# FraPria/proovread

Hardware: AMD Instinct MI355X
Metric: corrected long-read Mbases/sec per node (higher is better)
Workload: dtype int32

## Files before the change

### include/prgpu.h

```cpp
#ifndef PRGPU_H
#define PRGPU_H
#include <stdint.h>
#ifdef __cplusplus
extern "C" {
#endif

enum {
    PR_OK = 0,
    PR_ERR_ARG = -1,
    PR_ERR_HIP = -2,
    PR_ERR_SAM = -3,
    PR_ERR_NOSEQ = -4,
    PR_ERR_BIN_RANGE = -5,
    PR_ERR_DIV0 = -6,
    PR_ERR_CIGAR = -7,
    PR_ERR_BEYOND_REF = -8,
    PR_ERR_CAPACITY = -9,
    PR_ERR_UNSUPPORTED = -10,
};

const char *pr_last_error(void);
const char *pr_version(void);

typedef struct pr_ctx pr_ctx;
// ... 224 lines not shown
int pr_seed_map(const pr_seed_index *h, const pr_seed_opts *o, const uint8_t *sr_seq, const int64_t *sr_off,
                int n_sr, int n_threads, pr_seed_tasks *out);
void pr_seed_tasks_free(pr_seed_tasks *t);
int pr_seed_index_occ(const pr_seed_index *h, const uint8_t *s, int n, int64_t *count);
int pr_seed_index_digest(const pr_seed_index *h, uint64_t *out6);
int pr_seed_index_koff(const pr_seed_index *h, uint64_t *koff, uint64_t *ksplit);
int pr_seed_gpu_index_koff(pr_ctx *ctx, uint64_t *koff, uint64_t *ksplit);
int pr_seed_smem(const pr_seed_index *h, const uint8_t *q, int len, int x, int64_t min_intv, int32_t *start,
                 int32_t *end, int64_t *occ, int cap, int *n_out);
int pr_seed_gpu_upload(pr_ctx *ctx, const pr_seed_index *h);
int pr_seed_gpu_map(pr_ctx *ctx, const pr_seed_opts *o, const uint8_t *sr_seq, const int64_t *sr_off, int n_sr,
                    pr_seed_tasks *out, int32_t *status);
int pr_seed_gpu_index_build(pr_ctx *ctx, const uint8_t *lr_seq, const int64_t *lr_off, int n_lr);
int pr_seed_gpu_index_digest(pr_ctx *ctx, uint64_t *out6);
int pr_seed_gpu_index_last_ms(pr_ctx *ctx, double *ms);
int pr_seed_gpu_seed_count(pr_ctx *ctx, int64_t *n);
int pr_seed_gpu_seeds(pr_ctx *ctx, pr_seed_tasks *out);
int pr_seed_gpu_pass2_reads(pr_ctx *ctx, int64_t *n);
int pr_seed_gpu_pass_reads(pr_ctx *ctx, int64_t *n4);
int pr_seed_gpu_last_ms(pr_ctx *ctx, double *ms);
int pr_seed_gpu_phase_ticks(pr_ctx *ctx, uint64_t *ticks4);
int pr_seed_gpu_lane_ticks(pr_ctx *ctx, uint64_t *ticks6);
int pr_seed_gpu_occ_ticks(pr_ctx *ctx, uint64_t *ticks3);
int pr_seed_gpu_pass2_ticks(pr_ctx *ctx, uint64_t *t7);
int pr_seed_gpu_pass2_ms(pr_ctx *ctx, double *ms);
int pr_seed_map_device_caps(const pr_seed_index *h, const pr_seed_opts *o, const uint8_t *sr_seq,
                            const int64_t *sr_off, int n_sr, int n_threads, pr_seed_tasks *out, int32_t *status);
int pr_seed_map_device_pass1(const pr_seed_index *h, const pr_seed_opts *o, const uint8_t *sr_seq,
                             const int64_t *sr_off, int n_sr, int budget, pr_seed_tasks *out, int32_t *status,
                             int32_t *hits);

typedef struct pr_iter_batch {
    pr_sw_batch sw;
    const int64_t *task_lr_off;
    const uint8_t *lr_qual;
    const uint8_t *ref_seq;
} pr_iter_batch;
int pr_iter_upload(pr_ctx *ctx, const pr_iter_batch *b);
int pr_iter_upload_gpu_seeds(pr_ctx *ctx, const pr_iter_batch *b);
int pr_iter_launch(pr_ctx *ctx, const pr_sw_opts *o, const pr_cns_params *p);
int pr_iter_download(pr_ctx *ctx, pr_cns_out *out);
int pr_fmt_chim_lines(int32_t n_lr, const char *names, const int64_t *name_off, const int32_t *nchim,
                      const int64_t *chim_off, const int32_t *chim, char **text, int64_t *len, int64_t *n_lines);
int pr_iter_download_range(pr_ctx *ctx, int32_t first, int32_t n, pr_cns_out *out);
int pr_iter_bounds(pr_ctx *ctx, int32_t *n_lr, int64_t *n_task, pr_cns_bounds *bd);
int pr_iter_alignment_stats(pr_ctx *ctx, int64_t *n_aln, int64_t *sum_ncig, int64_t *sum_lseq);
// ... 171 lines not shown
```

### proovread_amd/csrc/seed_api.cpp

```cpp
#include <algorithm>
#include <climits>
#include <cstdio>
#include <cstdlib>
#include <cstring>
#include <vector>

#include "ctx.h"
#include "seed_index_dev.h"
#include "seed_plan.h"

static int seed_text4(pr_ctx *c, seedc::IndexView &v, hipStream_t s) {
    int rc = c->sd[SI_TEXT4].ensure((size_t)ix_pack4_words(v.n_text) * 8);
    if (rc) return rc;
    const int e = ix_pack4_launch(v.text, v.n_text, c->sd[SI_TEXT4].as<uint64_t>(), s);
    if (e) return set_error(PR_ERR_HIP, "text packing: %s", hipGetErrorString((hipError_t)e));
    v.text4 = c->sd[SI_TEXT4].as<uint64_t>();
    v.walk_nw = v.n_text > ((int64_t)64 << 24) ? 1 : 4;
    if (const char *w = getenv("PRGPU_SEED_WALK_NW"))
        v.walk_nw = atoi(w) == 1 ? 1 : 4;
    return 0;
}

static int upload_blk_fr(pr_ctx *c, seedc::IndexView &v, const int64_t *cstart, const int64_t *off, int n_lr,
                         int64_t l_pac, int64_t n_text, hipStream_t s) {
// ... 380 lines not shown
                          : 0;
}

int map_buffers(SeedMap &M, const pr_seed_opts *o, const uint8_t *sr_seq, bool in_sb_seq, const int64_t *sr_off) {
    pr_ctx *c = M.c;
    DevBuf *D = M.D;
    SeedDev &K = M.K;
    const int n_sr = M.n_sr;
    hipStream_t s = M.s;
    int rc;
    K.dp = nullptr;
    if (seedc::seed_flt_min_score(*o, M.qmax) >= 0) {
        if ((rc = D[SB_DP].ensure((size_t)M.waves * 2 * 201 * 64 * sizeof(int16_t)))) return rc;
        K.dp = D[SB_DP].as<int16_t>();
    }
    const int64_t scratch = std::max<int64_t>(M.waves * 64 * K.stride, M.lanes2 * seedc::scratch_bytes(M.caps));
    const int64_t nb = n_sr ? sr_off[n_sr] : 0;
    const int64_t slot_bytes = (int64_t)M.caps.out * (int64_t)sizeof(pr_seed_task);
    c->seed_sr_bases = nb;
    if ((!in_sb_seq && (rc = upload(D[SB_SEQ], sr_seq, (size_t)nb, s))) || (rc = upload(D[SB_OFF], sr_off, (size_t)n_sr + 1, s)) ||
        (rc = D[SB_SCRATCH].ensure((size_t)scratch)) ||
        (rc = D[SB_OUT].ensure((size_t)(std::min<int64_t>(M.chunk, n_sr) * slot_bytes + 16))) ||
        (rc = D[SB_NOUT].ensure((size_t)n_sr * 4 + 16)) || (rc = D[SB_STATUS].ensure((size_t)n_sr * 4 + 16)) ||
        (rc = D[SB_NEXT].ensure(256)) || (rc = D[SB_PRE].ensure(((size_t)n_sr + 1) * 8)) ||
        (rc = D[SB_DENSE].ensure(sizeof(pr_seed_task))) || (M.occ_words && (rc = D[SB_OCC].ensure((size_t)M.occ_words * 8))))
        return rc;
    K.sr_seq = D[SB_SEQ].as<uint8_t>();
    K.sr_off = D[SB_OFF].as<int64_t>();
    K.out = D[SB_OUT].as<pr_seed_task>();
    K.n_out = D[SB_NOUT].as<int32_t>();
    K.status = D[SB_STATUS].as<int32_t>();
    K.next = D[SB_NEXT].as<int32_t>();
    K.prof = reinterpret_cast<unsigned long long *>(D[SB_NEXT].as<uint8_t>() + 64);
    K.occ = seedc::OccPool{D[SB_OCC].as<uint64_t>(), reinterpret_cast<unsigned long long *>(K.next + 4), M.occ_words};
    HIPCHK(hipMemsetAsync(K.next, 0, 256, s));
    return 0;
}

int pass1(SeedMap &M, int64_t r0, int64_t r1, std::vector<int32_t> &redo, seedp::Flagged &f) {
    DevBuf *D = M.D;
    SeedDev &K = M.K;
    hipStream_t s = M.s;
    int rc;
    K.caps = M.small;
    K.caps.budget = M.budget;
    K.stride = seedc::scratch_bytes(M.small);
    K.n_lanes = M.waves;
    K.batch = 64;
    K.scratch = D[SB_SCRATCH].as<uint8_t>();
    K.rlist = nullptr;
    K.n_list = 0;
    K.out0 = r0;
    K.n_sr = r1;
    int32_t start = (int32_t)r0;
    const char *lpt = getenv("PRGPU_SEED_LPT");
    if (lpt && lpt[0] == '1') {
        int32_t *order = nullptr;
        if ((rc = D[SB_ORDER].ensure(seed_order_bytes(r1 - r0)))) return rc;
// ... 278 lines not shown
    if (!c || !ticks4) return set_error(PR_ERR_ARG, "null arg");
    if (!c->sd[SB_NEXT].p) return set_error(PR_ERR_ARG, "no pr_seed_gpu_map launch yet");
    HIPCHK(hipSetDevice(c->device));
    HIPCHK(hipMemcpy(ticks4, c->sd[SB_NEXT].as<uint8_t>() + 64, 32, hipMemcpyDeviceToHost));
    return 0;
}

extern "C" int pr_seed_gpu_lane_ticks(pr_ctx *c, uint64_t *ticks6) {
    if (!c || !ticks6) return set_error(PR_ERR_ARG, "null arg");
    if (!c->sd[SB_NEXT].p) return set_error(PR_ERR_ARG, "no pr_seed_gpu_map launch yet");
    HIPCHK(hipSetDevice(c->device));
    HIPCHK(hipMemcpy(ticks6, c->sd[SB_NEXT].as<uint8_t>() + 64 + 4 * 8, 48, hipMemcpyDeviceToHost));
    return 0;
}

extern "C" int pr_seed_gpu_pass2_ticks(pr_ctx *c, uint64_t *t7) {
    if (!c || !t7) return set_error(PR_ERR_ARG, "null arg");
    if (!c->sd[SB_NEXT].p) return set_error(PR_ERR_ARG, "no pr_seed_gpu_map launch yet");
    HIPCHK(hipSetDevice(c->device));
    HIPCHK(hipMemcpy(t7, c->sd[SB_NEXT].as<uint8_t>() + 64 + 13 * 8, 56, hipMemcpyDeviceToHost));
    return 0;
}

extern "C" int pr_seed_gpu_occ_ticks(pr_ctx *c, uint64_t *ticks3) {
    if (!c || !ticks3) return set_error(PR_ERR_ARG, "null arg");
    if (!c->sd[SB_NEXT].p) return set_error(PR_ERR_ARG, "no pr_seed_gpu_map launch yet");
    HIPCHK(hipSetDevice(c->device));
    HIPCHK(hipMemcpy(ticks3, c->sd[SB_NEXT].as<uint8_t>() + 64 + 10 * 8, 24, hipMemcpyDeviceToHost));
    return 0;
}
```

### proovread_amd/csrc/seed_chain.h

```cpp
#pragma once
#include "seed_core.h"

#if defined(__HIP_DEVICE_COMPILE__)
#define SCC_SYNC()                                              \
    do {                                                        \
        __builtin_amdgcn_fence(__ATOMIC_RELEASE, "wavefront");  \
        __builtin_amdgcn_wave_barrier();                        \
        __builtin_amdgcn_fence(__ATOMIC_ACQUIRE, "wavefront");  \
    } while (0)
#define SCC_LANES \
    for (int lane = (int)__builtin_amdgcn_mbcnt_hi(~0u, __builtin_amdgcn_mbcnt_lo(~0u, 0u)), go_ = 1; go_; go_ = 0)
#define SCC_END SCC_SYNC()
#define SCC_ADD(p, v) __hip_atomic_fetch_add(p, v, __ATOMIC_RELAXED, __HIP_MEMORY_SCOPE_WORKGROUP)
#define SCC_OR(p, v) __hip_atomic_fetch_or(p, v, __ATOMIC_RELAXED, __HIP_MEMORY_SCOPE_WORKGROUP)
namespace prgpu {
namespace seedc {
template <class T> __device__ inline T scc_cas(T *p, T c, T v) {
    __hip_atomic_compare_exchange_strong(p, &c, v, __ATOMIC_RELAXED, __ATOMIC_RELAXED, __HIP_MEMORY_SCOPE_WORKGROUP);
    return c;
}
}
}
#define SCC_CAS(p, c, v) ::prgpu::seedc::scc_cas(p, c, v)
#define SCC_NOW() __builtin_amdgcn_s_memrealtime()
#define SCC_STAT(L, k) ((void)0)
#else
#define SCC_STAT(L, k) (++(L).sv[k])
#define SCC_LANES for (int lane = 0; lane < 64; ++lane)
#define SCC_END ((void)0)
namespace prgpu {
namespace seedc {
template <class T> inline T scc_add(T *p, T v) { const T o = *p; *p = (T)(o + v); return o; }
template <class T> inline T scc_or(T *p, T v) { const T o = *p; *p = (T)(o | v); return o; }
template <class T> inline T scc_cas(T *p, T c, T v) { const T o = *p; if (o == c) *p = v; return o; }
}
}
#define SCC_ADD(p, v) ::prgpu::seedc::scc_add(p, v)
#define SCC_OR(p, v) ::prgpu::seedc::scc_or(p, v)
#define SCC_CAS(p, c, v) ::prgpu::seedc::scc_cas(p, c, v)
#define SCC_NOW() 0ULL
#endif

namespace prgpu {
namespace seedc {

constexpr int32_t OCC_MAX = 16384;
struct OccPool {
    uint64_t *w;
    unsigned long long *cursor;
    int64_t cap;
};
SC_HD constexpr int64_t occ_words(int n) { return (int64_t)n + (n + 1) / 2; }
SC_HD const uint32_t *occ_ql(const uint64_t *hfr, int n) { return reinterpret_cast<const uint32_t *>(hfr + n); }
SC_HD int32_t occ_words_per_read(bool lazy) { return lazy ? 384 : 3072; }

SC_HD int occ_taken(const pr_seed_opts &O, int64_t np) {
    const int64_t step = np > O.max_occ ? np / O.max_occ : 1;
// ... 65 lines not shown
    *first = w0;
    *n_occ = n;
    return 0;
}

template <int S, int HT, int CH>
struct ChainLds {
    static_assert(S % 8 == 0 && S < 32768 && CH % 64 == 0 && (HT & (HT - 1)) == 0, "slot indices are int16");
    static constexpr int SEEDS = S, RANGES = HT / 2;
    uint64_t hfr[S];
    uint32_t ql[S];
    int16_t nx[S];
    int16_t chead[S], ctail[S], cn[S];
    int16_t cnx[S];
    uint16_t cidx[S];
    int16_t ts[S];
    union {
        struct {
            int32_t key[HT];
            int16_t head[HT], tail[HT];
            uint64_t hfr[CH];
            uint32_t ql[CH];
            int16_t idx[CH];
            uint8_t own[CH];
        } ch;
        struct {
            int16_t pl[S];
            int16_t sch[S];
            int16_t kept[S];
            int16_t fm[S];
            int16_t kb[S], ke[S], kw[S];
        } po;
    } u;
    int32_t cnt[64], cur[64];
    int32_t sv[16];
    uint32_t mk[2][4];
};
enum {
    SV_ERR = 0, SV_NRG, SV_NP, SV_NK, SV_LARGE, SV_DROP, SV_NO, SV_STEP, SV_NS, SV_NC,
    SV_TIES, SV_INS_HEAD, SV_INS_MID, SV_INS_TAIL, SV_WR_LT
};

SC_HD uint32_t range_hash(int32_t key) { return (uint32_t)key * 0x9E3779B1u; }

template <int S, int HT, int CH>
SC_HD int chain_read(const IndexView &I, const pr_seed_opts &O, ChainLds<S, HT, CH> &L, const uint64_t *g_hfr,
                     const uint32_t *g_ql, int n, int len, int sid, pr_seed_task *out, int cap_out, int *n_out,
                     unsigned long long *ticks = nullptr, int lim_seeds = S, int lim_chains = S) {
    *n_out = 0;
    lim_seeds = lim_seeds < S ? lim_seeds : S;
    lim_chains = lim_chains < S ? lim_chains : S;
    if (n > OCC_MAX) return SC_OVER_SEEDS;
    if (n <= 0) return 0;
    unsigned long long t_last = ticks ? SCC_NOW() : 0ULL;
    (void)t_last;
#define SCC_TICK(k)                                     \
    do {                                                \
        if (ticks) {                                    \
            const unsigned long long t_ = SCC_NOW();    \
            ticks[k] += t_ - t_last;                    \
            t_last = t_;                                \
        }                                               \
    } while (0)
    const int64_t l_pac = I.l_pac;
    auto rbeg = [&L](int e) -> int64_t { return (int64_t)(L.hfr[e] >> FR_RID_BITS); };
    auto qb = [&L](int e) -> int { return (int)(L.ql[e] & 0xFFFFu); };
    auto sl = [&L](int e) -> int { return (int)(L.ql[e] >> 16); };

    SCC_LANES {
        if (lane < 16) L.sv[lane] = 0;
        if (lane < 8) L.mk[lane >> 2][lane & 3] = 0u;
        for (int k = lane; k < HT; k += 64) L.u.ch.key[k] = -1;
    }
    SCC_END;
    for (int c0 = 0; c0 < n && !L.sv[SV_ERR]; c0 += CH) {
        const int m = n - c0 < CH ? n - c0 : CH;
        SCC_LANES { L.cnt[lane] = 0; }
        SCC_END;
        SCC_LANES {
            for (int e = lane; e < m; e += 64) {
                const uint64_t v = g_hfr[c0 + e];
                L.u.ch.hfr[e] = v;
                L.u.ch.ql[e] = g_ql[c0 + e];
                const int rid = (int)(v & ((1u << FR_RID_BITS) - 1u));
                const int32_t key = rid * 2 + ((int64_t)(v >> FR_RID_BITS) >= l_pac ? 1 : 0);
                const int o = (int)(range_hash(key) >> 26);
                L.u.ch.own[e] = (uint8_t)o;
                SCC_ADD(&L.cnt[o], 1);
            }
            for (int e = m + lane; e < ((m + 7) & ~7); e += 64) L.u.ch.own[e] = 255;
        }
        SCC_END;
        SCC_LANES {
            int x = 0;
            for (int t = 0; t < lane; ++t) x += L.cnt[t];
            L.cur[lane] = x;
        }
        SCC_END;
        SCC_LANES {
            int c = L.cur[lane];
            for (int e0 = 0; e0 < m; e0 += 8) {
                uint64_t w;
                __builtin_memcpy(&w, L.u.ch.own + e0, 8);
#pragma unroll
                for (int u = 0; u < 8; ++u)
                    if ((int)((w >> (8 * u)) & 0xFF) == lane) L.u.ch.idx[c++] = (int16_t)(e0 + u);
            }
        }
        SCC_END;
        SCC_LANES {
            const int first = L.cur[lane], mine = L.cnt[lane];
            for (int t = 0; t < mine; ++t) {
                const int e = L.u.ch.idx[first + t];
                const uint64_t v = L.u.ch.hfr[e];
                const uint32_t qlv = L.u.ch.ql[e];
                const int64_t rb = (int64_t)(v >> FR_RID_BITS);
                const int rid = (int)(v & ((1u << FR_RID_BITS) - 1u));
                const int32_t key = rid * 2 + (rb >= l_pac ? 1 : 0);
                const int qbe = (int)(qlv & 0xFFFFu), sle = (int)(qlv >> 16);
                uint32_t h = range_hash(key) & (uint32_t)(HT - 1);
                bool found = false, claimed = false;
                for (int probe = 0; probe < HT; ++probe) {
                    const int32_t kk = L.u.ch.key[h];
                    if (kk == key) { found = true; break; }
                    if (kk == -1) {
                        const int32_t old = SCC_CAS(&L.u.ch.key[h], (int32_t)-1, key);
                        if (old == -1) { claimed = true; break; }
                        if (old == key) { found = true; break; }
                    }
                    h = (h + 1) & (uint32_t)(HT - 1);
                }
                if (claimed && SCC_ADD(&L.sv[SV_NRG], 1) >= HT / 2) claimed = false;
// ... 47 lines not shown
                L.cn[c] = 1;
                L.cidx[c] = (uint16_t)(c0 + e);
                if (!found) {
                    L.u.ch.head[h] = L.u.ch.tail[h] = (int16_t)c;
                    L.cnx[c] = -1;
                } else if (at < 0) {
                    L.cnx[c] = L.u.ch.head[h];
                    L.u.ch.head[h] = (int16_t)c;
                    SCC_STAT(L, SV_INS_HEAD);
                } else {
                    const int nxc = L.cnx[at];
                    L.cnx[c] = (int16_t)nxc;
                    L.cnx[at] = (int16_t)c;
                    if (nxc < 0) {
                        L.u.ch.tail[h] = (int16_t)c;
                        SCC_STAT(L, SV_INS_TAIL);
                    } else {
                        SCC_STAT(L, SV_INS_MID);
                    }
                }
            }
        }
        SCC_END;
    }
    if (L.sv[SV_ERR]) return L.sv[SV_ERR];
    SCC_TICK(0);
    const int ncv = L.sv[SV_NC];
    SCC_LANES {
        for (int c = lane; c < ncv; c += 64) {
            int64_t qe = 0, re = 0;
            int wq = 0, wr = 0;
            for (int k = L.chead[c]; k >= 0; k = L.nx[k]) {
                const int q0 = qb(k), ln = sl(k);
                const int64_t r0 = rbeg(k);
                if (q0 >= qe) wq += ln;
                else if (q0 + ln > qe) wq += (int)(q0 + ln - qe);
                qe = qe > q0 + ln ? qe : q0 + ln;
                if (r0 >= re) wr += ln;
                else if (r0 + ln > re) wr += (int)(r0 + ln - re);
                re = re > r0 + ln ? re : r0 + ln;
            }
            int w = wr < wq ? wr : wq;
            if (wr < wq) SCC_STAT(L, SV_WR_LT);
            w = w < 32767 ? w : 32767;
            L.cnx[c] = (int16_t)w;
        }
    }
    SCC_END;
    SCC_LANES {
        for (int c = lane; c < ncv; c += 64) {
            const int w = L.cnx[c];
            if (w >= O.min_chain_weight) {
                const int m = SCC_ADD(&L.sv[SV_NP], 1);
                L.u.po.pl[m] = (int16_t)c;
                L.u.po.kw[m] = (int16_t)w;
            }
        }
    }
    SCC_END;
    const int nch = L.sv[SV_NP];
    const bool keep_all = O.drop_ratio <= 0;
    SCC_LANES {
        for (int m = lane; m < nch; m += 64) {
            const int c = L.u.po.pl[m], w = L.u.po.kw[m];
            const int64_t ps = rbeg(L.chead[c]);
            const int ix = L.cidx[c];
            int rank = 0;
            for (int j = 0; j < nch; ++j) {
                const int wj = L.u.po.kw[j];
                if (wj > w) ++rank;
                else if (wj == w) {
                    const int cj = L.u.po.pl[j];
                    const int64_t pj = rbeg(L.chead[cj]);
                    rank += (pj < ps || (pj == ps && (int)L.cidx[cj] < ix)) ? 1 : 0;
                    if (pj == ps && cj != c) SCC_STAT(L, SV_TIES);
                }
            }
            L.u.po.sch[rank] = (int16_t)c;
            L.u.po.kept[rank] = keep_all ? 3 : 0;
        }
    }
    SCC_END;
    if (nch > 0 && !keep_all) {
        SCC_LANES {
            if (lane == 0) {
                const int c = L.u.po.sch[0], hd = L.chead[c], tl = L.ctail[c];
                const int w0 = L.cnx[c];
                L.u.po.kb[0] = (int16_t)qb(hd);
                L.u.po.ke[0] = (int16_t)(qb(tl) + sl(tl));
                L.u.po.kw[0] = (int16_t)w0;
                L.u.po.fm[0] = -1;
                L.u.po.kept[0] = 3;
                L.sv[SV_NK] = 1;
                L.sv[SV_LARGE] = L.sv[SV_DROP] = 0;
                L.sv[SV_STEP] = 0;
            }
        }
        SCC_END;
        for (int i = 1; i < nch; ++i) {
            const int ci = L.u.po.sch[i], hi = L.chead[ci], ti = L.ctail[ci];
            const int bi = qb(hi), ei = qb(ti) + sl(ti), wi = L.cnx[ci];
            for (int k0 = 0; k0 < L.sv[SV_NK] && !L.sv[SV_DROP]; k0 += 64) {
                const int set = L.sv[SV_STEP] & 1;
                SCC_LANES {
                    const int k = k0 + lane;
                    if (k < L.sv[SV_NK]) {
                        const int bj = L.u.po.kb[k], ej = L.u.po.ke[k], wj = L.u.po.kw[k];
                        const int bmax = bj > bi ? bj : bi;
                        const int emin = ej < ei ? ej : ei;
                        if (emin > bmax) {
                            const int li = ei - bi, lj = ej - bj;
                            const int minl = li < lj ? li : lj;
                            if (emin - bmax >= minl * O.mask_level && minl < O.max_chain_gap) {
                                SCC_OR(&L.mk[set][lane >> 5], 1u << (lane & 31));
                                if (wi < wj * O.drop_ratio && wj - wi >= O.min_seed_len << 1)
                                    SCC_OR(&L.mk[set][2 + (lane >> 5)], 1u << (lane & 31));
                            }
                        }
                    }
                }
                SCC_END;
                SCC_LANES {
                    const uint64_t ov = (uint64_t)L.mk[set][0] | ((uint64_t)L.mk[set][1] << 32);
                    const uint64_t br = (uint64_t)L.mk[set][2] | ((uint64_t)L.mk[set][3] << 32);
                    const int last = br ? ctz64(br) : 63;
                    const uint64_t seen = ov & (last >= 63 ? ~0ull : ((2ull << last) - 1ull));
                    if (((seen >> lane) & 1ull) && L.u.po.fm[k0 + lane] < 0) L.u.po.fm[k0 + lane] = (int16_t)i;
                    if (lane == 63) {
                        if (seen) L.sv[SV_LARGE] = 1;
                        if (br) L.sv[SV_DROP] = 1;
                        L.sv[SV_STEP] = set ^ 1;
                        L.mk[set ^ 1][0] = L.mk[set ^ 1][1] = L.mk[set ^ 1][2] = L.mk[set ^ 1][3] = 0u;
                    }
                }
                SCC_END;
            }
            SCC_LANES {
                if (lane == 0) {
                    if (!L.sv[SV_DROP]) {
                        const int nk = L.sv[SV_NK];
                        L.u.po.kb[nk] = (int16_t)bi;
                        L.u.po.ke[nk] = (int16_t)ei;
                        L.u.po.kw[nk] = (int16_t)wi;
                        L.u.po.fm[nk] = -1;
                        L.u.po.kept[i] = L.sv[SV_LARGE] ? 2 : 3;
                        L.sv[SV_NK] = nk + 1;
                    }
                    L.sv[SV_LARGE] = L.sv[SV_DROP] = 0;
                }
            }
            SCC_END;
        }
        SCC_LANES {
            for (int k = lane; k < L.sv[SV_NK]; k += 64)
                if (L.u.po.fm[k] >= 0) L.u.po.kept[L.u.po.fm[k]] = 1;
        }
        SCC_END;
    }
    SCC_TICK(1);
    SCC_LANES {
        if (lane == 0) {
            int no = 0, nkept = 0;
            for (int i = 0; i < nch; ++i) {
                if (L.u.po.kept[i] == 0) {
                    L.u.po.kb[i] = -1;
                    continue;
                }
                L.u.po.kb[i] = (int16_t)no;
                L.u.po.ke[i] = (int16_t)nkept++;
                no += L.cn[L.u.po.sch[i]];
            }
            L.sv[SV_NO] = no;
        }
    }
    SCC_END;
    const int no = L.sv[SV_NO];
    if (no > cap_out) return SC_OVER_OUT;
    SCC_LANES {
        for (int i = lane; i < nch; i += 64) {
            int t = L.u.po.kb[i];
            if (t < 0) continue;
            for (int k = L.chead[L.u.po.sch[i]]; k >= 0; k = L.nx[k], ++t) {
                L.ts[t] = (int16_t)k;
                L.u.po.pl[t] = (int16_t)i;
            }
        }
    }
    SCC_END;
    SCC_LANES {
        for (int t = lane; t < no; t += 64) {
            const int i = L.u.po.pl[t], k = L.ts[t];
            const int c = L.u.po.sch[i], first = L.u.po.kb[i], cnn = L.cn[c];
            const int hd = L.chead[c];
            const int ln = sl(k);
            int rank = 0;
            int64_t r0 = INT64_MAX, r1 = INT64_MIN;
            for (int u = first; u < first + cnn; ++u) {
                const int ku = L.ts[u];
                const int qu = qb(ku), lu = sl(ku);
// ... 6 lines not shown
            }
            const int rid = (int)(L.hfr[hd] & ((1u << FR_RID_BITS) - 1u));
            const bool rev = rbeg(hd) >= l_pac;
            const int64_t lo0 = I.lr_off[rid], lo1 = I.lr_off[rid + 1];
            const int64_t Lr = lo1 - lo0;
            const int64_t cs = rev ? l_pac + (l_pac - lo1) : lo0;
            r0 -= cs;
            r1 -= cs;
            pr_seed_task tk;
            tk.sr = sid;
            tk.lr = rid;
            tk.strand = rev ? 1 : 0;
            tk.qbeg = qb(k);
            tk.rbeg = (int32_t)(rbeg(k) - cs);
            tk.slen = ln;
            tk.rmax0 = (int32_t)(r0 > 0 ? r0 : 0);
            tk.rmax1 = (int32_t)(r1 < Lr ? r1 : Lr);
            tk.chain = L.u.po.ke[i];
            tk.rank = rank;
            out[first + rank] = tk;
        }
    }
    SCC_END;
    SCC_TICK(2);
#undef SCC_TICK
    *n_out = no;
    return 0;
}

using ChainLdsSmall = ChainLds<512, 512, 256>;
using ChainLdsLarge = ChainLds<1536, 2048, 256>;

struct ChainHost {
    ChainLdsSmall a;
    ChainLdsLarge b;
    uint64_t pool[occ_words(OCC_MAX)];
};
template <class LA, class LB>
SC_HD int map_read_chain2(const IndexView &I, const pr_seed_opts &O, Scratch &S, LA &La, LB &Lb, uint64_t *pool,
                          int64_t pool_words, const uint8_t *q, int len, int sid, pr_seed_task *out, int cap_out,
                          int *n_out) {
    *n_out = 0;
    if (seed_flt_min_score(O, len) >= 0) return map_read(I, O, S, q, len, sid, out, cap_out, n_out);
    int err = S.hend ? build_starts(I, S, q, len) : build_occ(I, S, q, len);
    if (err) return err;
    int nm = 0, nocc = 0;
    unsigned long long cursor = 0;
// ... 32 lines not shown
```

### proovread_amd/csrc/seed_kernels.hip

```cpp
#include <hip/hip_runtime.h>

#include <rocprim/device/device_radix_sort.hpp>

#include "seed_chain.h"
#include "seed_core.h"
#include "seed_dev.h"

namespace prgpu {

#ifndef SEED_WAVES_DEF
#define SEED_WAVES_DEF 4
#endif
#ifndef SEED_LMAX_DEF
#define SEED_LMAX_DEF 1024
#endif
constexpr int SEED_WAVES = SEED_WAVES_DEF;
constexpr int SEED_LMAX = SEED_LMAX_DEF;
#ifndef SEED_MINB
#define SEED_MINB 4
#endif
#ifndef SEED_WAVE_MINB
#define SEED_WAVE_MINB SEED_MINB
#endif
#ifndef OCC_U
// ... 953 lines not shown
    int nb = 0;
    const hipError_t e = walk_nw == 1 ? hipOccupancyMaxActiveBlocksPerMultiprocessor(&nb, seed_wave_kernel<1>, 64 * SEED_WAVES, 0)
                                      : hipOccupancyMaxActiveBlocksPerMultiprocessor(&nb, seed_wave_kernel<4>, 64 * SEED_WAVES, 0);
    if (e != hipSuccess || nb < 1)
        nb = 2;
    return nb * SEED_WAVES;
}

int seed_launch(const SeedDev &D, void *stream) {
    if (D.n_list <= 0) return 0;
    const int64_t blocks = (D.n_lanes + SEED_WAVES - 1) / SEED_WAVES;
    if (D.V.walk_nw == 1)
        hipLaunchKernelGGL(seed_wave_kernel<1>, dim3((unsigned)blocks), dim3(64 * SEED_WAVES), 0, (hipStream_t)stream, D);
    else
        hipLaunchKernelGGL(seed_wave_kernel<4>, dim3((unsigned)blocks), dim3(64 * SEED_WAVES), 0, (hipStream_t)stream, D);
    return (int)hipGetLastError();
}

template <class LDS, bool SECOND>
__global__ void __launch_bounds__(64) seed_chain_kernel(SeedDev D) {
    __shared__ LDS L;
    const int lane = threadIdx.x;
    const int64_t nlim = D.rlist ? D.n_list : D.n_sr - D.out0;
    unsigned long long ct[3] = {0ULL, 0ULL, 0ULL};
    for (;;) {
        int j0 = 0;
        if (lane == 0) j0 = atomicAdd(D.next + (SECOND ? 2 : 1), 64);
        j0 = __shfl(j0, 0, 64);
        if (j0 >= nlim) {
            if (D.prof && lane == 0)
                for (int k = 0; k < 3; ++k) atomicAdd(&D.prof[4 + 3 + k], ct[k] * 64ULL);
            break;
        }
        int my_i = -1, my_n = 0, my_len = 0;
        if (j0 + lane < nlim) {
            const int i = D.rlist ? D.rlist[j0 + lane] : (int)(D.out0 + j0 + lane);
            const int len = (int)(D.sr_off[i + 1] - D.sr_off[i]);
            const int n = D.n_out[i];
            if (len > 0 && D.status[i] == 0 && seedc::seed_flt_min_score(D.O, len) < 0 && (SECOND ? n < 0 : n > 0))
                my_i = i, my_n = SECOND ? -n - 1 : n, my_len = len;
        }
        unsigned long long todo = __ballot(my_i >= 0);
        while (todo) {
            const int src = __ffsll((long long)todo) - 1;
            todo &= todo - 1;
            const int i = __shfl(my_i, src, 64), n = __shfl(my_n, src, 64), len = __shfl(my_len, src, 64);
            pr_seed_task *slots = D.out + (int64_t)(i - D.out0) * D.caps.out;
            const int64_t w0 = *reinterpret_cast<const int64_t *>(slots);
            __builtin_amdgcn_wave_barrier();
            const uint64_t *hfr = D.occ.w + w0;
            int nt = 0;
            const int err = seedc::chain_read(D.V, D.O, L, hfr, seedc::occ_ql(hfr, n), n, len, i, slots, D.caps.out, &nt,
                                              D.prof && lane == 0 ? ct : nullptr, D.caps.seeds, D.caps.chains);
            if (lane == 0) {
// ... 67 lines not shown
```

### proovread_amd/seed.py

```python
from __future__ import annotations

import ctypes as C

import numpy as np

from . import _abi


class SeedOpts(C.Structure):
    _fields_ = [("min_seed_len", C.c_int), ("min_chain_weight", C.c_int), ("w", C.c_int),
                ("split_factor", C.c_double), ("split_width", C.c_int), ("max_mem_intv", C.c_int),
                ("max_occ", C.c_int), ("drop_ratio", C.c_double), ("max_chain_gap", C.c_int),
                ("mask_level", C.c_double), ("a", C.c_int), ("o_del", C.c_int), ("e_del", C.c_int),
                ("o_ins", C.c_int), ("e_ins", C.c_int), ("b", C.c_int)]


class SeedTask(C.Structure):
    _fields_ = [(k, C.c_int32) for k in ("sr", "lr", "strand", "qbeg", "rbeg", "slen", "rmax0", "rmax1",
                                          "chain", "rank")]


class SeedTasks(C.Structure):
    _fields_ = [("n", C.c_int64), ("t", C.POINTER(SeedTask))]

# ... 172 lines not shown
def _phase_ms(L, ctx) -> dict:
    t = np.zeros(4, np.uint64)
    _abi.check(L.pr_seed_gpu_phase_ticks(ctx.h, t.ctypes.data), "pr_seed_gpu_phase_ticks")
    n2 = C.c_int64()
    _abi.check(L.pr_seed_gpu_pass2_reads(ctx.h, C.byref(n2)), "pr_seed_gpu_pass2_reads")
    out = {k: round(float(v) / 1e5, 1) for k, v in
           zip(("occ_table", "lane_phase_and_pass2_smems", "pass2_chaining", "pass2_filter_out"), t)}
    out["pass2_reads"] = n2.value
    if hasattr(L, "pr_seed_gpu_pass_reads"):
        pr = np.zeros(4, np.int64)
        L.pr_seed_gpu_pass_reads.argtypes = [C.c_void_p, C.c_void_p]
        _abi.check(L.pr_seed_gpu_pass_reads(ctx.h, pr.ctypes.data), "pr_seed_gpu_pass_reads")
        out["pass_reads"] = dict(zip(("pass1b_lane", "pass1b_wave", "pass2", "later"), (int(v) for v in pr)))
    lt = np.zeros(6, np.uint64)
    L.pr_seed_gpu_lane_ticks.argtypes = [C.c_void_p, C.c_void_p]
    _abi.check(L.pr_seed_gpu_lane_ticks(ctx.h, lt.ctypes.data), "pr_seed_gpu_lane_ticks")
    out["pass1_lane_ms_summed"] = {k: round(float(v) / 1e5, 1) for k, v in
                                   zip(("smem_pass", "reseeding", "y_seeds_sort", "chaining", "chain_flt", "output"), lt)}
    if hasattr(L, "pr_seed_gpu_occ_ticks"):
        ot = np.zeros(3, np.uint64)
        L.pr_seed_gpu_occ_ticks.argtypes = [C.c_void_p, C.c_void_p]
        _abi.check(L.pr_seed_gpu_occ_ticks(ctx.h, ot.ctypes.data), "pr_seed_gpu_occ_ticks")
        out["occ_table_parts"] = {k: round(float(v) / 1e5, 1) for k, v in zip(("starts", "hits", "count_table"), ot)}
    if hasattr(L, "pr_seed_gpu_pass2_ticks"):
        t2 = np.zeros(7, np.uint64)
        L.pr_seed_gpu_pass2_ticks.argtypes = [C.c_void_p, C.c_void_p]
        _abi.check(L.pr_seed_gpu_pass2_ticks(ctx.h, t2.ctypes.data), "pr_seed_gpu_pass2_ticks")
        out["pass2_parts"] = {"one_lane_reads": int(t2[0])}
        out["pass2_parts"].update({k: round(float(v) / 1e5, 1) for k, v in
                                   zip(("chain_wave", "chain_one_lane", "chain_flt", "max_read_occ_table",
                                        "max_read_smems", "max_read"), t2[1:])})
    p2 = C.c_double()
    _abi.check(L.pr_seed_gpu_pass2_ms(ctx.h, C.byref(p2)), "pr_seed_gpu_pass2_ms")
    out["pass2_wall_ms"] = round(p2.value, 1)
    return out


def _map_gpu(L, ctx, sr_seq, sr_off, opts, allow_flagged, keep_on_device=False):
    opts = opts or default_opts()
    sr_seq = np.ascontiguousarray(sr_seq, np.uint8)
    sr_off = np.ascontiguousarray(sr_off, np.int64)
    st = np.zeros(max(1, len(sr_off) - 1), np.int32)
    if keep_on_device:
        rc = L.pr_seed_gpu_map(ctx.h, C.byref(opts), sr_seq.ctypes.data, sr_off.ctypes.data, len(sr_off) - 1,
                               None, st.ctypes.data)
        if rc != 0 and not (allow_flagged and rc == -9):
# ... 45 lines not shown
```

Measured before the change: 239.0.

## Replace LDS atomics and serial loops in wave chaining with ballot/readlane primitives

Adds lane-register, ballot, readlane broadcast and prefix-scan primitives to the wave-level chaining kernel. It uses them to rewrite the owner bucketing (ballot match instead of LDS atomic counting and byte scans, with the next chunk prefetched into registers), the rank sort (keys broadcast across lanes instead of O(n^2) per-lane LDS reads), the drop pass (first 64 kept chains held in registers and masks built by ballot instead of LDS mask words and barriers), and the output-base computation (wave scan instead of a lane-0 serial loop). It also adds finer profiling tick counters and a host API to read them. The aim is to cut LDS traffic, barriers and serial single-lane work in the chaining phase, at the cost of more register pressure and more complex control flow.

```diff
diff --git a/include/prgpu.h b/include/prgpu.h
--- a/include/prgpu.h
+++ b/include/prgpu.h
@@ -270,6 +270,7 @@
 int pr_seed_gpu_phase_ticks(pr_ctx *ctx, uint64_t *ticks4);
 int pr_seed_gpu_lane_ticks(pr_ctx *ctx, uint64_t *ticks6);
 int pr_seed_gpu_occ_ticks(pr_ctx *ctx, uint64_t *ticks3);
+int pr_seed_gpu_chain_ticks(pr_ctx *ctx, uint64_t *ticks7);
 int pr_seed_gpu_pass2_ticks(pr_ctx *ctx, uint64_t *t7);
 int pr_seed_gpu_pass2_ms(pr_ctx *ctx, double *ms);
 int pr_seed_map_device_caps(const pr_seed_index *h, const pr_seed_opts *o, const uint8_t *sr_seq,
diff --git a/proovread_amd/csrc/seed_api.cpp b/proovread_amd/csrc/seed_api.cpp
--- a/proovread_amd/csrc/seed_api.cpp
+++ b/proovread_amd/csrc/seed_api.cpp
@@ -426,7 +426,7 @@
         (rc = D[SB_SCRATCH].ensure((size_t)scratch)) ||
         (rc = D[SB_OUT].ensure((size_t)(std::min<int64_t>(M.chunk, n_sr) * slot_bytes + 16))) ||
         (rc = D[SB_NOUT].ensure((size_t)n_sr * 4 + 16)) || (rc = D[SB_STATUS].ensure((size_t)n_sr * 4 + 16)) ||
-        (rc = D[SB_NEXT].ensure(256)) || (rc = D[SB_PRE].ensure(((size_t)n_sr + 1) * 8)) ||
+        (rc = D[SB_NEXT].ensure(512)) || (rc = D[SB_PRE].ensure(((size_t)n_sr + 1) * 8)) ||
         (rc = D[SB_DENSE].ensure(sizeof(pr_seed_task))) || (M.occ_words && (rc = D[SB_OCC].ensure((size_t)M.occ_words * 8))))
         return rc;
     K.sr_seq = D[SB_SEQ].as<uint8_t>();
@@ -437,7 +437,7 @@
     K.next = D[SB_NEXT].as<int32_t>();
     K.prof = reinterpret_cast<unsigned long long *>(D[SB_NEXT].as<uint8_t>() + 64);
     K.occ = seedc::OccPool{D[SB_OCC].as<uint64_t>(), reinterpret_cast<unsigned long long *>(K.next + 4), M.occ_words};
-    HIPCHK(hipMemsetAsync(K.next, 0, 256, s));
+    HIPCHK(hipMemsetAsync(K.next, 0, 512, s));
     return 0;
 }
 
@@ -762,6 +762,14 @@
     return 0;
 }
 
+extern "C" int pr_seed_gpu_chain_ticks(pr_ctx *c, uint64_t *ticks7) {
+    if (!c || !ticks7) return set_error(PR_ERR_ARG, "null arg");
+    if (!c->sd[SB_NEXT].p) return set_error(PR_ERR_ARG, "no pr_seed_gpu_map launch yet");
+    HIPCHK(hipSetDevice(c->device));
+    HIPCHK(hipMemcpy(ticks7, c->sd[SB_NEXT].as<uint8_t>() + 64 + 24 * 8, 56, hipMemcpyDeviceToHost));
+    return 0;
+}
+
 extern "C" int pr_seed_gpu_occ_ticks(pr_ctx *c, uint64_t *ticks3) {
     if (!c || !ticks3) return set_error(PR_ERR_ARG, "null arg");
     if (!c->sd[SB_NEXT].p) return set_error(PR_ERR_ARG, "no pr_seed_gpu_map launch yet");
diff --git a/proovread_amd/csrc/seed_chain.h b/proovread_amd/csrc/seed_chain.h
--- a/proovread_amd/csrc/seed_chain.h
+++ b/proovread_amd/csrc/seed_chain.h
@@ -24,6 +24,34 @@
 #define SCC_CAS(p, c, v) ::prgpu::seedc::scc_cas(p, c, v)
 #define SCC_NOW() __builtin_amdgcn_s_memrealtime()
 #define SCC_STAT(L, k) ((void)0)
+namespace prgpu {
+namespace seedc {
+__device__ inline int scc_lane() { return (int)__builtin_amdgcn_mbcnt_hi(~0u, __builtin_amdgcn_mbcnt_lo(~0u, 0u)); }
+template <class T> struct LaneReg {
+    T v;
+    __device__ T &at(int) { return v; }
+    __device__ const T &at(int) const { return v; }
+};
+template <class F> __device__ inline uint64_t scc_ballot(F f) { return __builtin_amdgcn_ballot_w64(f(scc_lane()) ? true : false); }
+__device__ inline int scc_bcast(const LaneReg<int> &r, int src) { return __builtin_amdgcn_readlane(r.v, src); }
+__device__ inline uint64_t scc_bcast(const LaneReg<uint64_t> &r, int src) {
+    const uint32_t lo = (uint32_t)__builtin_amdgcn_readlane((int)(uint32_t)r.v, src);
+    const uint32_t hi = (uint32_t)__builtin_amdgcn_readlane((int)(uint32_t)(r.v >> 32), src);
+    return (uint64_t)hi << 32 | lo;
+}
+template <class F> __device__ inline int scc_scan(LaneReg<int> &ex, F f) {
+    const int lane = scc_lane(), v = f(lane);
+    int x = v;
+#pragma unroll
+    for (int d = 1; d < 64; d <<= 1) {
+        const int y = __builtin_amdgcn_ds_bpermute((lane - d) << 2, x);
+        if (lane >= d) x += y;
+    }
+    ex.v = x - v;
+    return __builtin_amdgcn_readlane(x, 63);
+}
+}
+}
 #else
 #define SCC_STAT(L, k) (++(L).sv[k])
 #define SCC_LANES for (int lane = 0; lane < 64; ++lane)
@@ -33,6 +61,24 @@
 template <class T> inline T scc_add(T *p, T v) { const T o = *p; *p = (T)(o + v); return o; }
 template <class T> inline T scc_or(T *p, T v) { const T o = *p; *p = (T)(o | v); return o; }
 template <class T> inline T scc_cas(T *p, T c, T v) { const T o = *p; if (o == c) *p = v; return o; }
+template <class T> struct LaneReg {
+    T v[64];
+    T &at(int lane) { return v[lane]; }
+    const T &at(int lane) const { return v[lane]; }
+};
+template <class F> inline uint64_t scc_ballot(F f) {
+    uint64_t m = 0;
+    for (int lane = 0; lane < 64; ++lane) m |= f(lane) ? 1ull << lane : 0ull;
+    return m;
+}
+inline int scc_bcast(const LaneReg<int> &r, int src) { return r.v[src & 63]; }
+inline uint64_t scc_bcast(const LaneReg<uint64_t> &r, int src) { return r.v[src & 63]; }
+template <class F> inline int scc_scan(LaneReg<int> &ex, F f) {
+    int v[64], x = 0;
+    for (int lane = 0; lane < 64; ++lane) v[lane] = f(lane);
+    for (int lane = 0; lane < 64; ++lane) ex.v[lane] = x, x += v[lane];
+    return x;
+}
 }
 }
 #define SCC_ADD(p, v) ::prgpu::seedc::scc_add(p, v)
@@ -144,7 +190,6 @@
             uint64_t hfr[CH];
             uint32_t ql[CH];
             int16_t idx[CH];
-            uint8_t own[CH];
         } ch;
         struct {
             int16_t pl[S];
@@ -156,12 +201,13 @@
     } u;
     int32_t cnt[64], cur[64];
     int32_t sv[16];
-    uint32_t mk[2][4];
 };
 enum {
-    SV_ERR = 0, SV_NRG, SV_NP, SV_NK, SV_LARGE, SV_DROP, SV_NO, SV_STEP, SV_NS, SV_NC,
+    SV_ERR = 0, SV_NRG, SV_NP, SV_NS, SV_NC,
     SV_TIES, SV_INS_HEAD, SV_INS_MID, SV_INS_TAIL, SV_WR_LT
 };
+
+enum { CT_LOAD = 0, CT_LANES, CT_WEIGHTS, CT_SORT, CT_DROP, CT_BASE, CT_TASKS, CT_N };
 
 SC_HD uint32_t range_hash(int32_t key) { return (uint32_t)key * 0x9E3779B1u; }
 
@@ -191,45 +237,81 @@
 
     SCC_LANES {
         if (lane < 16) L.sv[lane] = 0;
-        if (lane < 8) L.mk[lane >> 2][lane & 3] = 0u;
         for (int k = lane; k < HT; k += 64) L.u.ch.key[k] = -1;
     }
     SCC_END;
+    constexpr int G = CH / 64;
+    LaneReg<uint64_t> nh[G];
+    LaneReg<uint32_t> nq[G];
+    auto fetch = [&](int c0) {
+        SCC_LANES {
+#pragma unroll
+            for (int g = 0; g < G; ++g) {
+                const int e = c0 + g * 64 + lane;
+                nh[g].at(lane) = e < n ? g_hfr[e] : 0ull;
+                nq[g].at(lane) = e < n ? g_ql[e] : 0u;
+            }
+        }
+    };
+    fetch(0);
     for (int c0 = 0; c0 < n && !L.sv[SV_ERR]; c0 += CH) {
         const int m = n - c0 < CH ? n - c0 : CH;
-        SCC_LANES { L.cnt[lane] = 0; }
+        LaneReg<int> own[G], pos[G], add[G], cur;
+        SCC_LANES {
+            L.cnt[lane] = 0;
+#pragma unroll
+            for (int g = 0; g < G; ++g) {
+                const int e = g * 64 + lane;
+                own[g].at(lane) = -1;
+                pos[g].at(lane) = add[g].at(lane) = 0;
+                if (e < m) {
+                    const uint64_t v = nh[g].at(lane);
+                    L.u.ch.hfr[e] = v;
+                    L.u.ch.ql[e] = nq[g].at(lane);
+                    const int rid = (int)(v & ((1u << FR_RID_BITS) - 1u));
+                    const int32_t key = rid * 2 + ((int64_t)(v >> FR_RID_BITS) >= l_pac ? 1 : 0);
+                    own[g].at(lane) = (int)(range_hash(key) >> 26);
+                }
+            }
+        }
+        SCC_END;
+        if (c0 + CH < n) fetch(c0 + CH);
+#pragma unroll
+        for (int g = 0; g < G; ++g) {
+            if (g * 64 >= m) break;
+            uint64_t bit[6];
+#pragma unroll
+            for (int b = 0; b < 6; ++b) bit[b] = scc_ballot([&](int lane) { return (own[g].at(lane) >> b) & 1; });
+            const uint64_t valid = scc_ballot([&](int lane) { return own[g].at(lane) >= 0; });
+            SCC_LANES {
+                const int o = own[g].at(lane);
+                if (o >= 0) {
+                    uint64_t same = valid;
+#pragma unroll
+                    for (int b = 0; b < 6; ++b) same &= ((o >> b) & 1) ? bit[b] : ~bit[b];
+                    const int before = __builtin_popcountll(same & ((1ull << lane) - 1ull));
+                    pos[g].at(lane) = L.cnt[o] + before;
+                    add[g].at(lane) = before ? 0 : __builtin_popcountll(same);
+                }
+            }
+            SCC_END;
+            SCC_LANES {
+                if (add[g].at(lane)) L.cnt[own[g].at(lane)] += add[g].at(lane);
+            }
+            SCC_END;
+        }
+        scc_scan(cur, [&](int lane) { return (int)L.cnt[lane]; });
+        SCC_LANES { L.cur[lane] = cur.at(lane); }
         SCC_END;
         SCC_LANES {
-            for (int e = lane; e < m; e += 64) {
-                const uint64_t v = g_hfr[c0 + e];
-                L.u.ch.hfr[e] = v;
-                L.u.ch.ql[e] = g_ql[c0 + e];
-                const int rid = (int)(v & ((1u << FR_RID_BITS) - 1u));
-                const int32_t key = rid * 2 + ((int64_t)(v >> FR_RID_BITS) >= l_pac ? 1 : 0);
-                const int o = (int)(range_hash(key) >> 26);
-                L.u.ch.own[e] = (uint8_t)o;
-                SCC_ADD(&L.cnt[o], 1);
-            }
-            for (int e = m + lane; e < ((m + 7) & ~7); e += 64) L.u.ch.own[e] = 255;
+#pragma unroll
+            for (int g = 0; g < G; ++g) {
+                const int o = own[g].at(lane);
+                if (o >= 0) L.u.ch.idx[L.cur[o] + pos[g].at(lane)] = (int16_t)(g * 64 + lane);
+            }
         }
         SCC_END;
-        SCC_LANES {
-            int x = 0;
-            for (int t = 0; t < lane; ++t) x += L.cnt[t];
-            L.cur[lane] = x;
-        }
-        SCC_END;
-        SCC_LANES {
-            int c = L.cur[lane];
-            for (int e0 = 0; e0 < m; e0 += 8) {
-                uint64_t w;
-                __builtin_memcpy(&w, L.u.ch.own + e0, 8);
-#pragma unroll
-                for (int u = 0; u < 8; ++u)
-                    if ((int)((w >> (8 * u)) & 0xFF) == lane) L.u.ch.idx[c++] = (int16_t)(e0 + u);
-            }
-        }
-        SCC_END;
+        SCC_TICK(CT_LOAD);
         SCC_LANES {
             const int first = L.cur[lane], mine = L.cnt[lane];
             for (int t = 0; t < mine; ++t) {
@@ -323,9 +405,9 @@
             }
         }
         SCC_END;
+        SCC_TICK(CT_LANES);
     }
     if (L.sv[SV_ERR]) return L.sv[SV_ERR];
-    SCC_TICK(0);
     const int ncv = L.sv[SV_NC];
     SCC_LANES {
         for (int c = lane; c < ncv; c += 64) {
@@ -354,128 +436,163 @@
             if (w >= O.min_chain_weight) {
                 const int m = SCC_ADD(&L.sv[SV_NP], 1);
                 L.u.po.pl[m] = (int16_t)c;
-                L.u.po.kw[m] = (int16_t)w;
+                L.ts[m] = (int16_t)w;
             }
         }
     }
     SCC_END;
     const int nch = L.sv[SV_NP];
+    SCC_TICK(CT_WEIGHTS);
     const bool keep_all = O.drop_ratio <= 0;
-    SCC_LANES {
-        for (int m = lane; m < nch; m += 64) {
-            const int c = L.u.po.pl[m], w = L.u.po.kw[m];
-            const int64_t ps = rbeg(L.chead[c]);
-            const int ix = L.cidx[c];
-            int rank = 0;
-            for (int j = 0; j < nch; ++j) {
-                const int wj = L.u.po.kw[j];
-                if (wj > w) ++rank;
-                else if (wj == w) {
-                    const int cj = L.u.po.pl[j];
-                    const int64_t pj = rbeg(L.chead[cj]);
-                    rank += (pj < ps || (pj == ps && (int)L.cidx[cj] < ix)) ? 1 : 0;
-                    if (pj == ps && cj != c) SCC_STAT(L, SV_TIES);
-                }
-            }
-            L.u.po.sch[rank] = (int16_t)c;
-            L.u.po.kept[rank] = keep_all ? 3 : 0;
+    auto sort_key = [&](int m, uint64_t &a, int &x) {
+        a = ~0ull, x = 0;
+        if (m < nch) {
+            const int c = L.u.po.pl[m];
+            a = (uint64_t)(32767 - L.ts[m]) << 40 | (uint64_t)rbeg(L.chead[c]);
+            x = L.cidx[c];
+        }
+    };
+    for (int m0 = 0; m0 < nch; m0 += 64) {
+        LaneReg<uint64_t> ka, ja;
+        LaneReg<int> kx, jx, rk;
+        SCC_LANES {
+            sort_key(m0 + lane, ka.at(lane), kx.at(lane));
+            rk.at(lane) = 0;
+        }
+        for (int j0 = 0; j0 < nch; j0 += 64) {
+            const int mj = nch - j0 < 64 ? nch - j0 : 64;
+            SCC_LANES { sort_key(j0 + lane, ja.at(lane), jx.at(lane)); }
+            for (int jj = 0; jj < mj; ++jj) {
+                const uint64_t a = scc_bcast(ja, jj);
+                const int x = scc_bcast(jx, jj);
+                SCC_LANES {
+                    rk.at(lane) += (a < ka.at(lane) || (a == ka.at(lane) && x < kx.at(lane))) ? 1 : 0;
+                    if (a == ka.at(lane) && j0 + jj != m0 + lane) SCC_STAT(L, SV_TIES);
+                }
+            }
+        }
+        SCC_LANES {
+            const int m = m0 + lane;
+            if (m < nch) {
+                const int c = L.u.po.pl[m], rank = rk.at(lane);
+                L.u.po.sch[rank] = (int16_t)c;
+                L.u.po.kept[rank] = keep_all ? 3 : 0;
+                if (!keep_all) {
+                    const int tl = L.ctail[c];
+                    L.u.po.kb[rank] = (int16_t)qb(L.chead[c]);
+                    L.u.po.ke[rank] = (int16_t)(qb(tl) + sl(tl));
+                    L.u.po.kw[rank] = L.ts[m];
+                }
+            }
         }
     }
     SCC_END;
+    SCC_TICK(CT_SORT);
     if (nch > 0 && !keep_all) {
-        SCC_LANES {
-            if (lane == 0) {
-                const int c = L.u.po.sch[0], hd = L.chead[c], tl = L.ctail[c];
-                const int w0 = L.cnx[c];
-                L.u.po.kb[0] = (int16_t)qb(hd);
-                L.u.po.ke[0] = (int16_t)(qb(tl) + sl(tl));
-                L.u.po.kw[0] = (int16_t)w0;
-                L.u.po.fm[0] = -1;
-                L.u.po.kept[0] = 3;
-                L.sv[SV_NK] = 1;
-                L.sv[SV_LARGE] = L.sv[SV_DROP] = 0;
-                L.sv[SV_STEP] = 0;
-            }
-        }
-        SCC_END;
-        for (int i = 1; i < nch; ++i) {
-            const int ci = L.u.po.sch[i], hi = L.chead[ci], ti = L.ctail[ci];
-            const int bi = qb(hi), ei = qb(ti) + sl(ti), wi = L.cnx[ci];
-            for (int k0 = 0; k0 < L.sv[SV_NK] && !L.sv[SV_DROP]; k0 += 64) {
-                const int set = L.sv[SV_STEP] & 1;
-                SCC_LANES {
-                    const int k = k0 + lane;
-                    if (k < L.sv[SV_NK]) {
-                        const int bj = L.u.po.kb[k], ej = L.u.po.ke[k], wj = L.u.po.kw[k];
-                        const int bmax = bj > bi ? bj : bi;
-                        const int emin = ej < ei ? ej : ei;
-                        if (emin > bmax) {
-                            const int li = ei - bi, lj = ej - bj;
-                            const int minl = li < lj ? li : lj;
-                            if (emin - bmax >= minl * O.mask_level && minl < O.max_chain_gap) {
-                                SCC_OR(&L.mk[set][lane >> 5], 1u << (lane & 31));
-                                if (wi < wj * O.drop_ratio && wj - wi >= O.min_seed_len << 1)
-                                    SCC_OR(&L.mk[set][2 + (lane >> 5)], 1u << (lane & 31));
+        LaneReg<int> rb, re, rw, rfm;
+        LaneReg<int> cb, ce, cw, cv;
+        SCC_LANES { rb.at(lane) = re.at(lane) = rw.at(lane) = 0, rfm.at(lane) = -1; }
+        int nk = 0;
+        for (int i0 = 0; i0 < nch; i0 += 64) {
+            const int mi = nch - i0 < 64 ? nch - i0 : 64;
+            SCC_LANES {
+                const bool in = lane < mi;
+                cb.at(lane) = in ? L.u.po.kb[i0 + lane] : 0;
+                ce.at(lane) = in ? L.u.po.ke[i0 + lane] : 0;
+                cw.at(lane) = in ? L.u.po.kw[i0 + lane] : 0;
+                cv.at(lane) = 0;
+            }
+            SCC_END;
+            for (int j = 0; j < mi; ++j) {
+                const int i = i0 + j;
+                const int bi = scc_bcast(cb, j), ei = scc_bcast(ce, j), wi = scc_bcast(cw, j);
+                bool large = false, drop = false;
+                for (int k0 = 0; k0 < nk && !drop; k0 += 64) {
+                    LaneReg<int> hit;
+                    SCC_LANES {
+                        const int k = k0 + lane;
+                        int h = 0;
+                        if (k < nk) {
+                            const int bj = k0 ? L.u.po.kb[k] : rb.at(lane), ej = k0 ? L.u.po.ke[k] : re.at(lane);
+                            const int wj = k0 ? L.u.po.kw[k] : rw.at(lane);
+                            const int bmax = bj > bi ? bj : bi;
+                            const int emin = ej < ei ? ej : ei;
+                            if (emin > bmax) {
+                                const int li = ei - bi, lj = ej - bj;
+                                const int minl = li < lj ? li : lj;
+                                if (emin - bmax >= minl * O.mask_level && minl < O.max_chain_gap) {
+                                    h = 1;
+                                    if (wi < wj * O.drop_ratio && wj - wi >= O.min_seed_len << 1) h = 3;
+                                }
+                            }
+                        }
+                        hit.at(lane) = h;
+                    }
+                    const uint64_t ov = scc_ballot([&](int lane) { return hit.at(lane) & 1; });
+                    const uint64_t br = scc_ballot([&](int lane) { return hit.at(lane) & 2; });
+                    const int last = br ? ctz64(br) : 63;
+                    const uint64_t seen = ov & (last >= 63 ? ~0ull : ((2ull << last) - 1ull));
+                    SCC_LANES {
+                        if ((seen >> lane) & 1ull) {
+                            if (k0 == 0) {
+                                if (rfm.at(lane) < 0) rfm.at(lane) = i;
+                            } else if (L.u.po.fm[k0 + lane] < 0) {
+                                L.u.po.fm[k0 + lane] = (int16_t)i;
                             }
                         }
                     }
-                }
-                SCC_END;
+                    large = large || seen != 0;
+                    drop = br != 0;
+                }
+                if (drop) continue;
                 SCC_LANES {
-                    const uint64_t ov = (uint64_t)L.mk[set][0] | ((uint64_t)L.mk[set][1] << 32);
-                    const uint64_t br = (uint64_t)L.mk[set][2] | ((uint64_t)L.mk[set][3] << 32);
-                    const int last = br ? ctz64(br) : 63;
-                    const uint64_t seen = ov & (last >= 63 ? ~0ull : ((2ull << last) - 1ull));
-                    if (((seen >> lane) & 1ull) && L.u.po.fm[k0 + lane] < 0) L.u.po.fm[k0 + lane] = (int16_t)i;
-                    if (lane == 63) {
-                        if (seen) L.sv[SV_LARGE] = 1;
-                        if (br) L.sv[SV_DROP] = 1;
-                        L.sv[SV_STEP] = set ^ 1;
-                        L.mk[set ^ 1][0] = L.mk[set ^ 1][1] = L.mk[set ^ 1][2] = L.mk[set ^ 1][3] = 0u;
-                    }
-                }
-                SCC_END;
-            }
-            SCC_LANES {
-                if (lane == 0) {
-                    if (!L.sv[SV_DROP]) {
-                        const int nk = L.sv[SV_NK];
+                    if (lane == j) cv.at(lane) = large ? 2 : 3;
+                    if (nk < 64) {
+                        if (lane == nk) rb.at(lane) = bi, re.at(lane) = ei, rw.at(lane) = wi, rfm.at(lane) = -1;
+                    } else if (lane == 0 && nk < S) {
                         L.u.po.kb[nk] = (int16_t)bi;
                         L.u.po.ke[nk] = (int16_t)ei;
                         L.u.po.kw[nk] = (int16_t)wi;
                         L.u.po.fm[nk] = -1;
-                        L.u.po.kept[i] = L.sv[SV_LARGE] ? 2 : 3;
-                        L.sv[SV_NK] = nk + 1;
                     }
-                    L.sv[SV_LARGE] = L.sv[SV_DROP] = 0;
-                }
+                }
+                if (nk >= 64) SCC_END;
+                ++nk;
+            }
+            SCC_LANES {
+                if (lane < mi && cv.at(lane)) L.u.po.kept[i0 + lane] = (int16_t)cv.at(lane);
             }
             SCC_END;
         }
         SCC_LANES {
-            for (int k = lane; k < L.sv[SV_NK]; k += 64)
+            if (lane < nk && rfm.at(lane) >= 0) L.u.po.kept[rfm.at(lane)] = 1;
+            for (int k = 64 + lane; k < nk && k < S; k += 64)
                 if (L.u.po.fm[k] >= 0) L.u.po.kept[L.u.po.fm[k]] = 1;
         }
         SCC_END;
     }
-    SCC_TICK(1);
-    SCC_LANES {
-        if (lane == 0) {
-            int no = 0, nkept = 0;
-            for (int i = 0; i < nch; ++i) {
-                if (L.u.po.kept[i] == 0) {
-                    L.u.po.kb[i] = -1;
-                    continue;
-                }
-                L.u.po.kb[i] = (int16_t)no;
-                L.u.po.ke[i] = (int16_t)nkept++;
-                no += L.cn[L.u.po.sch[i]];
-            }
-            L.sv[SV_NO] = no;
-        }
+    SCC_TICK(CT_DROP);
+    int no = 0, nkept = 0;
+    for (int i0 = 0; i0 < nch; i0 += 64) {
+        LaneReg<int> ex;
+        const int tot = scc_scan(ex, [&](int lane) {
+            const int i = i0 + lane;
+            return i < nch && L.u.po.kept[i] != 0 ? (int)L.cn[L.u.po.sch[i]] : 0;
+        });
+        const uint64_t kp = scc_ballot([&](int lane) { return i0 + lane < nch && L.u.po.kept[i0 + lane] != 0; });
+        SCC_LANES {
+            const int i = i0 + lane;
+            if (i < nch) {
+                const bool mine = (kp >> lane) & 1ull;
+                L.u.po.kb[i] = (int16_t)(mine ? no + ex.at(lane) : -1);
+                if (mine) L.u.po.ke[i] = (int16_t)(nkept + __builtin_popcountll(kp & ((1ull << lane) - 1ull)));
+            }
+        }
+        no += tot;
+        nkept += __builtin_popcountll(kp);
     }
     SCC_END;
-    const int no = L.sv[SV_NO];
+    SCC_TICK(CT_BASE);
     if (no > cap_out) return SC_OVER_OUT;
     SCC_LANES {
         for (int i = lane; i < nch; i += 64) {
@@ -528,7 +645,7 @@
         }
     }
     SCC_END;
-    SCC_TICK(2);
+    SCC_TICK(CT_TASKS);
 #undef SCC_TICK
     *n_out = no;
     return 0;
diff --git a/proovread_amd/csrc/seed_kernels.hip b/proovread_amd/csrc/seed_kernels.hip
--- a/proovread_amd/csrc/seed_kernels.hip
+++ b/proovread_amd/csrc/seed_kernels.hip
@@ -999,14 +999,19 @@
     __shared__ LDS L;
     const int lane = threadIdx.x;
     const int64_t nlim = D.rlist ? D.n_list : D.n_sr - D.out0;
-    unsigned long long ct[3] = {0ULL, 0ULL, 0ULL};
+    unsigned long long ct[seedc::CT_N] = {};
     for (;;) {
         int j0 = 0;
         if (lane == 0) j0 = atomicAdd(D.next + (SECOND ? 2 : 1), 64);
         j0 = __shfl(j0, 0, 64);
         if (j0 >= nlim) {
-            if (D.prof && lane == 0)
-                for (int k = 0; k < 3; ++k) atomicAdd(&D.prof[4 + 3 + k], ct[k] * 64ULL);
+            if (D.prof && lane == 0) {
+                using namespace seedc;
+                atomicAdd(&D.prof[7], (ct[CT_LOAD] + ct[CT_LANES]) * 64ULL);
+                atomicAdd(&D.prof[8], (ct[CT_WEIGHTS] + ct[CT_SORT] + ct[CT_DROP]) * 64ULL);
+                atomicAdd(&D.prof[9], (ct[CT_BASE] + ct[CT_TASKS]) * 64ULL);
+                for (int k = 0; k < CT_N; ++k) atomicAdd(&D.prof[24 + k], ct[k] * 64ULL);
+            }
             break;
         }
         int my_i = -1, my_n = 0, my_len = 0;
diff --git a/proovread_amd/seed.py b/proovread_amd/seed.py
--- a/proovread_amd/seed.py
+++ b/proovread_amd/seed.py
@@ -218,6 +218,13 @@
         L.pr_seed_gpu_occ_ticks.argtypes = [C.c_void_p, C.c_void_p]
         _abi.check(L.pr_seed_gpu_occ_ticks(ctx.h, ot.ctypes.data), "pr_seed_gpu_occ_ticks")
         out["occ_table_parts"] = {k: round(float(v) / 1e5, 1) for k, v in zip(("starts", "hits", "count_table"), ot)}
+    if hasattr(L, "pr_seed_gpu_chain_ticks"):
+        ct = np.zeros(7, np.uint64)
+        L.pr_seed_gpu_chain_ticks.argtypes = [C.c_void_p, C.c_void_p]
+        _abi.check(L.pr_seed_gpu_chain_ticks(ctx.h, ct.ctypes.data), "pr_seed_gpu_chain_ticks")
+        out["chain_kernel_ms_summed"] = {k: round(float(v) / 1e5, 1) for k, v in
+                                         zip(("load_owner_lists", "lane_chaining", "weights_listing", "rank_sort", "drop_pass",
+                                              "task_base", "tasks"), ct)}
     if hasattr(L, "pr_seed_gpu_pass2_ticks"):
         t2 = np.zeros(7, np.uint64)
         L.pr_seed_gpu_pass2_ticks.argtypes = [C.c_void_p, C.c_void_p]
```

After: 249.1, median of 6. +4.2%, better.
